# js43o/HifiDiff

Measured on AMD Instinct MI355X. Metric: faces/sec (whole node), 16→128 1000-step reverse diffusion, batch 64, higher is better.
Workload: dtype bf16

## Files before the change

hifidiff_amd/_lib.py:

```python
import ctypes
import os
import subprocess

import torch

_HERE = os.path.dirname(os.path.abspath(__file__))
LIB_PATH = os.path.join(_HERE, "libhifidiff_hip.so")
UNITS = [os.path.join(_HERE, "csrc", f) for f in ("hd_lib.hip", "hd_aux.hip", "hd_stages.hip", "hd_stages_rows.hip", "hd_strip.hip", "hd_dispatch_ln.hip", "hd_dispatch_lnface.hip", "hd_dispatch_bf16.hip", "hd_dispatch_misc.hip")]
SOURCES = UNITS + [os.path.join(_HERE, "csrc", f) for f in ("hd_gemm.hpp", "hd_dispatch.hpp", "hd_kernels.hpp", "hd_chain.hpp", "hd_conv.hpp", "hd_cr.hpp", "hd_vae.hpp", "hd_internal.hpp", "hd_faceset.hpp", "hd_stage_api.hpp", "hd_xcd.hpp", "hd_xcd2.hpp", "hd_face.hpp", "hd_strip.hpp", "hd_wide.hpp", "hd_end.hpp", "hd_color.hpp")]
HEADER = os.path.join(os.path.dirname(_HERE), "include", "hifidiff_hip.h")


def unit_deps(unit):
    import re
    seen, todo = [], [unit]
    while todo:
        f = os.path.normpath(todo.pop())
        if f in seen or not os.path.exists(f):
            continue
        seen.append(f)
        with open(f) as fh:
            for inc in re.findall(r'^\s*#include\s+"([^"]+)"', fh.read(), flags=re.M):
                todo.append(os.path.join(os.path.dirname(f), inc))
    return seen

EXPORTS = [
    "hd_create", "hd_create_unconditional", "hd_prepare_unconditional", "hd_cr_create", "hd_cr_forward", "hd_vae_create", "hd_vae_encode", "hd_vae_decode", "hd_destroy", "hd_last_error", "hd_load_weights", "hd_finalize_weights", "hd_prepare",
    "hd_prepare_from_priors", "hd_fpg", "hd_idc", "hd_eps", "hd_sample", "hd_sample_multistep", "hd_sample_rows", "hd_sample_rows_multistep", "hd_prepare_slots",
    "hd_pool_config", "hd_pool_prepare", "hd_pool_commit",
    "hd_sample_faces", "hd_sample_faces_multistep", "hd_sample_spans", "hd_mask_faces", "hd_guide_config", "hd_guide_faces", "hd_color_fix", "hd_preview_config", "hd_preview_read", "hd_scheduler_step",
    "hd_scheduler_step_multistep", "hd_num_ops", "hd_num_chains",
    "hd_debug_limit_ops", "hd_debug_op_name", "hd_debug_op_info", "hd_debug_read_op", "hd_debug_read", "hd_debug_write", "hd_set_option", "hd_get_option", "hd_check",
    "hd_set_profiling", "hd_get_profile",
]


class TensorDesc(ctypes.Structure):
    _fields_ = [("name", ctypes.c_char_p), ("data", ctypes.c_void_p), ("ndim", ctypes.c_int32),
                ("shape", ctypes.c_int64 * 4), ("is_device", ctypes.c_int32)]


class Schedule(ctypes.Structure):
    _fields_ = [("n_steps", ctypes.c_int32), ("timesteps", ctypes.POINTER(ctypes.c_float)),
                ("coef", ctypes.POINTER(ctypes.c_float))]


class ScheduleMS(ctypes.Structure):
    _fields_ = [("n_steps", ctypes.c_int32), ("timesteps", ctypes.POINTER(ctypes.c_float)),
                ("coef", ctypes.POINTER(ctypes.c_float))]


def build(force=False, verbose=False):
    if not force and os.path.exists(LIB_PATH):
        newest = max(os.path.getmtime(p) for p in SOURCES + [HEADER])
        if os.path.getmtime(LIB_PATH) >= newest:
            return LIB_PATH
    hipcc = os.environ.get("HIPCC", "/opt/rocm/bin/hipcc")
    flags = ["--offload-arch=gfx950", "-O3", "-std=c++17", "-fPIC", "-Wno-unused-result", "-Wno-unused-function"]
    objdir = os.path.join(_HERE, "csrc", "build")
    os.makedirs(objdir, exist_ok=True)
    objs = [os.path.join(objdir, os.path.splitext(os.path.basename(u))[0] + ".o") for u in UNITS]
    stale = [(u, o) for u, o in zip(UNITS, objs)
             if force or not os.path.exists(o) or os.path.getmtime(o) < max(os.path.getmtime(d) for d in unit_deps(u))]
    cmds = [[hipcc] + flags + ["-c", u, "-o", o] for u, o in stale]
    if verbose:
        for c in cmds:
            print(" ".join(c))
    procs = [subprocess.Popen(c) for c in cmds]
    failed = [u for (u, _), pr in zip(stale, procs) if pr.wait() != 0]
    if failed:
        raise subprocess.CalledProcessError(1, "hipcc -c " + " ".join(os.path.basename(f) for f in failed))
    link = [hipcc, "--offload-arch=gfx950", "-shared", "-fPIC", "-o", LIB_PATH] + objs
    if verbose:
        print(" ".join(link))
    subprocess.run(link, check=True)
    return LIB_PATH


_lib = None


def lib():
    global _lib
    if _lib is not None:
        return _lib
    if not os.path.exists(LIB_PATH):
        raise RuntimeError(f"{LIB_PATH} is not built (no CPU fallback exists); run __graft_entry__.build()")
    L = ctypes.CDLL(LIB_PATH)
    vp, i32, i64, u64 = ctypes.c_void_p, ctypes.c_int, ctypes.c_int64, ctypes.c_uint64
    L.hd_create.argtypes = [ctypes.POINTER(vp), i32, i32]
    L.hd_create_unconditional.argtypes = [ctypes.POINTER(vp), i32, i32]
    L.hd_prepare_unconditional.argtypes = [vp, i32, vp]
# ... 68 lines not shown
```

hifidiff_amd/csrc/hd_chain.hpp:

```cpp
#pragma once
#include "hd_gemm.hpp"

namespace hd {

struct ChainP {
    int M, hw, face0;
    const unsigned short* G;
    const float* pooled;
    const float* pool_part; int pool_nparts; float pool_scale; float* pooled_out;
    const float* X;
    const uint4 *Wsca, *W3, *W4, *W5;
    const float *bsca, *b3, *b4, *b5, *beta, *gamma;
    const float* film;
    int film_face_stride, film_gain_off, film_bias_off;
    float ln_eps;
    float* Xout;
    unsigned short* Xout16;
    float2* stats_out;
    unsigned short* outg16;
    const float *gate_c, *gate_s, *add_src;
#ifdef HD_STAMPS
    unsigned long long* stamps;
#endif
};
#ifdef HD_STAMPS
#define HD_CSTAMP(i) do { if (p.stamps && threadIdx.x == 0) p.stamps[(size_t)blockIdx.x * 8 + (i)] = __builtin_amdgcn_s_memrealtime(); } while (0)
#else
#define HD_CSTAMP(i) do { } while (0)
#endif

template <int C, int MT_ = 1>
struct ChainCfg {
    static constexpr int NT = C / 32;
    static constexpr int MT = MT_;
    static constexpr int WAVES = NT, THREADS = 64 * WAVES, BM = 32 * MT;
    static constexpr int TPW = 1;
    static constexpr int KS = C / 16;
    static constexpr int AROW = C * 2 + 16;
    static constexpr int YROW = C + 4;
    static constexpr int A1_OFF = 0;
    static constexpr int A2_OFF = A1_OFF + BM * AROW;
    static constexpr int Y_OFF = A2_OFF + BM * AROW;
    static constexpr int S_OFF = Y_OFF + BM * YROW * 4;
    static constexpr int GB_OFF = S_OFF + C * 4;
    static constexpr int SMEM = GB_OFF + 2 * C * 4;
    static_assert(TPW >= 1, "C must be a multiple of 128");
};

template <int C>
__device__ __forceinline__ void chain_load_b(const uint4* W, int tile, int lane, uint4* b) {
    const uint4* Wl = W + (size_t)tile * ChainCfg<C>::KS * 64 + lane;
#pragma unroll
    for (int ks = 0; ks < ChainCfg<C>::KS; ++ks) b[ks] = Wl[ks * 64];
}
template <int C, int MT>
__device__ __forceinline__ void chain_mma(const char* sA, const uint4* b, int lane, f32x16_t (&acc)[MT]) {
    const char* ap = sA + (lane & 31) * ChainCfg<C>::AROW + (lane >> 5) * 16;
#pragma unroll
    for (int mt = 0; mt < MT; ++mt)
#pragma unroll
        for (int i = 0; i < 16; ++i) acc[mt][i] = 0.f;
#pragma unroll
    for (int ks = 0; ks < ChainCfg<C>::KS; ++ks)
#pragma unroll
        for (int mt = 0; mt < MT; ++mt)
            acc[mt] = __builtin_amdgcn_mfma_f32_32x32x16_bf16(*reinterpret_cast<const bf16x8_t*>(ap + mt * 32 * ChainCfg<C>::AROW + ks * 32),
                                                              __builtin_bit_cast(bf16x8_t, b[ks]), acc[mt], 0, 0, 0);
}

#ifndef HD_CHAIN_OCC
#define HD_CHAIN_OCC 3
#endif
template <int C, int MT>
__global__ __launch_bounds__((ChainCfg<C, MT>::THREADS), (C == 128 && MT == 1 ? HD_CHAIN_OCC : 1)) void naf_chain_kernel(const ChainP p) {
    typedef ChainCfg<C, MT> K;
    extern __shared__ __attribute__((aligned(16))) char smem[];
    const int tid = threadIdx.x, lane = tid & 63, wave = tid >> 6;
    const int row0 = blockIdx.x * K::BM;
    const int face = row0 / p.hw;
    float* s_vec = reinterpret_cast<float*>(smem + K::S_OFF);
    float* gb = reinterpret_cast<float*>(smem + K::GB_OFF);
    float* yt = reinterpret_cast<float*>(smem + K::Y_OFF);
    const int tile = wave;
    const int col = tile * 32 + (lane & 31);
    const bool full = row0 + K::BM <= p.M;

    HD_CSTAMP(0);
    uint4 bw[K::KS], bw2[K::KS];
    chain_load_b<C>(p.Wsca, tile, lane, bw);
    chain_load_b<C>(p.W3, tile, lane, bw2);
    {
        const float* f = p.film + (size_t)(p.face0 + face) * p.film_face_stride;
        for (int k = tid; k < C; k += K::THREADS) { gb[k] = f[p.film_gain_off + k]; gb[C + k] = f[p.film_bias_off + k]; }
    }
    const float c_bsca = p.bsca[col], c_b3 = p.b3[col], c_beta = p.beta[col], c_b4a = p.b4[col], c_b4b = p.b4[col + C], c_b5 = p.b5[col],
                c_gamma = p.gamma[col];
    constexpr int kGIt = K::BM * (C / 8) / K::THREADS;
    static_assert(kGIt * K::THREADS == K::BM * (C / 8), "G tile / threads");
    uint4 gx[kGIt];
#pragma unroll
    for (int it = 0; it < kGIt; ++it) {
        const int u = tid + it * K::THREADS;
        const int rl = u / (C / 8), kq = u - rl * (C / 8);
        const int row = (full || row0 + rl < p.M) ? row0 + rl : row0;
        gx[it] = *reinterpret_cast<const uint4*>(p.G + (size_t)row * C + kq * 8);
    }
    {
        float* pl = yt;
        const float* pv = p.pooled + (size_t)face * C;
        if (p.pool_part) {
            const float* pp = p.pool_part + (size_t)face * p.pool_nparts * C;
            for (int k = tid; k < C; k += K::THREADS) {
                float v[8], s = 0.f;
#pragma unroll
                for (int b = 0; b < 8; ++b) v[b] = b < p.pool_nparts ? pp[b * C + k] : 0.f;
#pragma unroll
                for (int b = 0; b < 8; ++b) s += v[b];
                pl[k] = s * p.pool_scale;
                if (row0 == face * p.hw) p.pooled_out[(size_t)face * C + k] = pl[k];
            }
        } else {
            for (int k = tid; k < C; k += K::THREADS) pl[k] = pv[k];
        }
        __syncthreads();
        uint4 a[K::KS];
#pragma unroll
        for (int ks = 0; ks < K::KS; ++ks) {
            const float* q = pl + ks * 16 + 8 * (lane >> 5);
            const float4 v0 = *reinterpret_cast<const float4*>(q), v1 = *reinterpret_cast<const float4*>(q + 4);
            const uint4 row0 = make_uint4(pack2(v0.x, v0.y), pack2(v0.z, v0.w), pack2(v1.x, v1.y), pack2(v1.z, v1.w));
            a[ks] = (lane & 31) == 0 ? row0 : make_uint4(0, 0, 0, 0);
// ... 180 lines not shown
```

hifidiff_amd/csrc/hd_face.hpp:

```cpp
#pragma once
#ifndef HD_FACE_ROWS
#define HD_FACE_ROWS 0
#endif
#if HD_FACE_ROWS
#define HD_FACE_KERNEL naf_face_rows_stage_kernel
#define HD_FACE_LAUNCH launch_face_rows_stage
#else
#define HD_FACE_KERNEL naf_face_stage_kernel
#define HD_FACE_LAUNCH launch_face_stage
#endif
#include "hd_chain.hpp"
#include "hd_xcd.hpp"

namespace hd {

#ifdef HD_STAMPS
#define HD_FSTAMP(i) do { if (p.stamps && tid == 0) p.stamps[((size_t)blk * gridDim.x + blockIdx.x) * 8 + (i)] = __builtin_amdgcn_s_memrealtime(); } while (0)
#else
#define HD_FSTAMP(i) do { } while (0)
#endif

template <int C, int OWN_ = 32>
struct FaceCfg {
    static constexpr int S = (C == 128) ? 16 : 8;
    static constexpr int OWN = OWN_;
    static constexpr int HW = S * S, CL = HW / OWN, RI = OWN / S;
    static constexpr int NT = C / 32, THREADS = 64 * NT, KS = C / 16;
    static constexpr int ROWS = OWN + 2 * S, MT1 = (ROWS + 31) / 32;
    static constexpr int AROW = C * 2 + 16;
    static constexpr int XROW = C + 4;
    static constexpr int XT_OFF = 0;
    static constexpr int ALN_OFF = XT_OFF + OWN * XROW * 4;
    static constexpr int A1_OFF = ALN_OFF + 32 * AROW;
    static constexpr int T1_OFF = ALN_OFF + 64 * AROW;
    static constexpr int SV_OFF = T1_OFF + NT * MT1 * 32 * 32 * 4;
    static constexpr int GB_OFF = SV_OFF + C * 4;
    static constexpr int PL_OFF = GB_OFF + 4 * C * 4;
    static constexpr int PP_OFF = PL_OFF + C * 4;
    static constexpr int SMEM = PP_OFF + C * 4;
    static_assert(ROWS <= 64 && (OWN == 32 || OWN == 16) && RI >= 2 && RI % 2 == 0, "own + halo rows fit two MFMA row tiles; two lane halves share the image rows");
};

typedef __attribute__((address_space(1))) unsigned fs_gu32;

template <int C>
__device__ __forceinline__ void face_load_b(const uint4* W, int tile, int lane, uint4* b) {
#ifdef HD_STAMPS
    if (!W) return;
#endif
    const uint4* Wl = W + (size_t)tile * (C / 16) * 64 + lane;
#pragma unroll
    for (int ks = 0; ks < C / 16; ++ks) b[ks] = xs_ldg_u4(Wl + ks * 64);
}

template <int C, int OWN = 32>
__global__ __launch_bounds__((FaceCfg<C, OWN>::THREADS), 2) void HD_FACE_KERNEL(const FStageP p) {
    typedef FaceCfg<C, OWN> K;
    extern __shared__ __attribute__((aligned(16))) char smem[];
    __shared__ XBlockW s_blk[XS_MAXBLK];
    __shared__ unsigned s_abort, s_base;
    const int tid = threadIdx.x, lane = tid & 63, wave = __builtin_amdgcn_readfirstlane(tid >> 6);
    const int bid = blockIdx.x, xcd = bid & 7, jj = bid >> 3;
    const int fl = jj / K::CL, kk = jj - fl * K::CL;
    const int face = xcd * 8 + fl;
    if (face >= p.B) return;
    const int M = p.B * K::HW;
    const int row0 = face * K::HW + kk * OWN;
    const bool has_up = kk > 0, has_dn = kk < K::CL - 1;
    const int tile = wave, col = tile * 32 + (lane & 31);
    float* xt = reinterpret_cast<float*>(smem + K::XT_OFF);
    float* s_vec = reinterpret_cast<float*>(smem + K::SV_OFF);
    float* gb = reinterpret_cast<float*>(smem + K::GB_OFF);
    float* pooled = reinterpret_cast<float*>(smem + K::PL_OFF);
    float* poolp = reinterpret_cast<float*>(smem + K::PP_OFF);
    float* t1w = reinterpret_cast<float*>(smem + K::T1_OFF) + wave * K::MT1 * 32 * 32;

    {
        const unsigned* src = reinterpret_cast<const unsigned*>(p.blocks);
        unsigned* dst = reinterpret_cast<unsigned*>(s_blk);
        for (int i = tid; i < p.nblocks * (int)(sizeof(XBlockW) / 4); i += K::THREADS) dst[i] = src[i];
        if (tid == 0) {
            s_abort = __hip_atomic_load((fs_gu32*)p.abort_dev, __ATOMIC_RELAXED, __HIP_MEMORY_SCOPE_AGENT);
            s_base = __hip_atomic_load((fs_gu32*)(p.gstate + face * 16), __ATOMIC_RELAXED, __HIP_MEMORY_SCOPE_AGENT) * 64u;
        }
    }
    const __amdgpu_buffer_rsrc_t rs_X = __builtin_amdgcn_make_buffer_rsrc(p.X, 0, (int)((size_t)M * C * 4), 0x00020000);
    const __amdgpu_buffer_rsrc_t rs_PP = __builtin_amdgcn_make_buffer_rsrc(p.pool_part, 0, p.B * K::CL * C * 4, 0x00020000);
    fs_gu32* flags = (fs_gu32*)(p.flags + face * 16);

    bool intro = false;
    float* hb = reinterpret_cast<float*>(smem + K::T1_OFF);
    if constexpr (C == 128 && OWN == 32) intro = p.intro_lat != nullptr;
    bool from_x = !intro;
    if constexpr (C == 256 && OWN == 16) from_x = p.down_A == nullptr;
    if (from_x) {
// ... 124 lines not shown
                uint4 v = make_uint4(0, 0, 0, 0);
                if (ok) {
                    const int l0row = face * 256 + (2 * y1 + (tap >> 1)) * 16 + 2 * x1 + (tap & 1);
                    v = *reinterpret_cast<const uint4*>(p.down_A + (size_t)l0row * 128 + q * 8);
                }
                *reinterpret_cast<uint4*>(sA + r * DROW + (tap * 128 + q * 8) * 2) = v;
            }
            uint4 wa[16], wb[16];
            {
                const uint4* Wl = p.down_W + (size_t)tile * 32 * 64 + lane;
#pragma unroll
                for (int ks = 0; ks < 16; ++ks) wa[ks] = xs_ldg_u4(Wl + ks * 64);
#pragma unroll
                for (int ks = 0; ks < 16; ++ks) wb[ks] = xs_ldg_u4(Wl + (16 + ks) * 64);
            }
            const float bias = p.down_b[col];
            __syncthreads();
            f32x16_t acc;
#pragma unroll
            for (int i = 0; i < 16; ++i) acc[i] = 0.f;
            const char* ap = sA + (lane & 31) * DROW + (lane >> 5) * 16;
#pragma unroll
            for (int ks = 0; ks < 16; ++ks)
                acc = __builtin_amdgcn_mfma_f32_32x32x16_bf16(*reinterpret_cast<const bf16x8_t*>(ap + ks * 32), __builtin_bit_cast(bf16x8_t, wa[ks]), acc, 0, 0, 0);
#pragma unroll
            for (int ks = 0; ks < 16; ++ks)
                acc = __builtin_amdgcn_mfma_f32_32x32x16_bf16(*reinterpret_cast<const bf16x8_t*>(ap + (16 + ks) * 32), __builtin_bit_cast(bf16x8_t, wb[ks]), acc, 0, 0, 0);
#pragma unroll
            for (int i = 0; i < 16; ++i) {
                const int r = (i & 3) + 8 * (i >> 2) + 4 * (lane >> 5);
                float* dst = r < OWN ? xt + r * K::XROW : hb + (r - OWN) * K::XROW;
                dst[col] = acc[i] + bias;
            }
        }
    }
    __syncthreads();
    const unsigned base = s_base;
    bool dead = false;

    auto publish = [&](unsigned value) __attribute__((always_inline)) {
        asm volatile("s_waitcnt vmcnt(0)" ::: "memory");
        __syncthreads();
        if (tid == 0) __hip_atomic_store(flags + kk, value, __ATOMIC_RELAXED, __HIP_MEMORY_SCOPE_AGENT);
    };
    auto poll = [&](unsigned value, unsigned code) __attribute__((always_inline)) {
        if (wave == 0) {
            for (unsigned spins = 0;; ++spins) {
                const unsigned v = lane < K::CL ? __hip_atomic_load(flags + lane, __ATOMIC_RELAXED, __HIP_MEMORY_SCOPE_AGENT) : value;
                if (__all((int)(v - value) >= 0)) break;
                if (spins > XS_SPINS) {
                    if (lane == 0) {
                        s_abort = 1u;
                        __hip_atomic_store((fs_gu32*)p.abort_dev, code, __ATOMIC_RELAXED, __HIP_MEMORY_SCOPE_AGENT);
                        __hip_atomic_store((fs_gu32*)p.tmo, code, __ATOMIC_RELAXED, __HIP_MEMORY_SCOPE_SYSTEM);
                    }
                    break;
                }
                __builtin_amdgcn_s_sleep(1);
            }
        }
    };
    auto wait_for = [&](unsigned value, unsigned code) __attribute__((always_inline)) {
        if (wave == 0) {
            for (unsigned spins = 0;; ++spins) {
                const unsigned v = lane < K::CL ? __hip_atomic_load(flags + lane, __ATOMIC_RELAXED, __HIP_MEMORY_SCOPE_AGENT) : value;
                const bool inject = p.test_abort >= 1000 && (int)(code & 0xffu) == p.test_abort - 1000 && face == 0;
                if (!inject && __all((int)(v - value) >= 0)) break;
                if (spins > XS_SPINS || inject) {
                    if (lane == 0) {
                        s_abort = 1u;
                        __hip_atomic_store((fs_gu32*)p.abort_dev, code, __ATOMIC_RELAXED, __HIP_MEMORY_SCOPE_AGENT);
                        __hip_atomic_store((fs_gu32*)p.tmo, code, __ATOMIC_RELAXED, __HIP_MEMORY_SCOPE_SYSTEM);
                    }
                    break;
                }
                __builtin_amdgcn_s_sleep(1);
            }
        }
        __syncthreads();
        dead = s_abort != 0u;
    };
    constexpr int V4 = C / 64;
    auto ln_row = [&](const float4 (&v)[V4], const float* g, const float* b, char* dst_row, bool valid) __attribute__((always_inline)) {
        const int l16 = lane & 15;
        float sum = 0.f;
#pragma unroll
        for (int i = 0; i < V4; ++i) sum += (v[i].x + v[i].y) + (v[i].z + v[i].w);
        const float mean = row16_sum(sum) * (1.0f / C);
        float q = 0.f;
#pragma unroll
        for (int i = 0; i < V4; ++i) {
            const float d0 = v[i].x - mean, d1 = v[i].y - mean, d2 = v[i].z - mean, d3 = v[i].w - mean;
            q += (d0 * d0 + d1 * d1) + (d2 * d2 + d3 * d3);
        }
        const float rstd = 1.0f / sqrtf(row16_sum(q) * (1.0f / C) + p.ln_eps);
        const float nmr = -mean * rstd;
#pragma unroll
        for (int i = 0; i < V4; ++i) {
            const int k = 4 * l16 + 64 * i;
            const float x4[4] = {v[i].x, v[i].y, v[i].z, v[i].w};
            float o[4];
#pragma unroll
            for (int e = 0; e < 4; ++e) {
                const float xq = bf16_bits_to_f32(f32_to_bf16_bits(x4[e]));
                o[e] = valid ? fmaf(fmaf(xq, rstd, nmr), g[k + e], b[k + e]) : 0.f;
            }
            *reinterpret_cast<uint2*>(dst_row + k * 2) = make_uint2(pack2(o[0], o[1]), pack2(o[2], o[3]));
        }
    };

    const int nb_run = p.block_limit < 0 ? 0 : (p.block_limit > 0 && p.block_limit < p.nblocks) ? p.block_limit : p.nblocks;
    uint4 bw[K::KS], bw2[K::KS];
    for (int blk = 0; blk < nb_run; ++blk) {
        const XBlockW& B = s_blk[blk];
        HD_FSTAMP(0);
        float4 gbv = make_float4(0.f, 0.f, 0.f, 0.f);
        const int gi = tid - 64;
        static_assert(K::THREADS - 64 >= C, "one float4 of the FiLM rows per thread of waves 1..");
#if HD_FACE_ROWS
        if (gi >= 0 && gi < C) gbv = *reinterpret_cast<const float4*>(p.film + (size_t)face * p.film_face_stride + B.film_off + 4 * gi);
#else
        if (gi >= 0 && gi < C) gbv = *reinterpret_cast<const float4*>(p.film + B.film_off + 4 * gi);
#endif
        face_load_b<C>(B.w1, tile, lane, bw);
        if constexpr (C == 128) face_load_b<C>(B.w1, tile + K::NT, lane, bw2);
        constexpr bool kEarly = C == 128;
        float c_b1a = 0.f, c_b1b = 0.f, dwa[9], dwb[9], dba = 0.f, dbb = 0.f;
        auto load_dw_consts = [&]() __attribute__((always_inline)) {
            c_b1a = xs_ldg_f(B.b1 + col); c_b1b = xs_ldg_f(B.b1 + col + C);
#pragma unroll
            for (int t = 0; t < 9; ++t) { dwa[t] = xs_ldg_f(B.dw_w + (size_t)t * 2 * C + col); dwb[t] = xs_ldg_f(B.dw_w + (size_t)t * 2 * C + col + C); }
            dba = xs_ldg_f(B.dw_b + col); dbb = xs_ldg_f(B.dw_b + col + C);
        };
        if constexpr (kEarly) load_dw_consts();
        if (blk > 0) poll(base + 2u * (unsigned)(blk - 1) + 2u, 0x200u + (unsigned)blk);
        if (gi >= 0 && gi < C) *reinterpret_cast<float4*>(gb + 4 * gi) = gbv;
        __syncthreads();
        if (s_abort) return;
        {
            const int l16 = lane & 15;
            constexpr int ROWS = K::ROWS;
            constexpr int HRI = (ROWS - OWN + K::NT * 4 - 1) / (K::NT * 4);
            constexpr int HSH = (K::NT * 4 - OWN % (K::NT * 4)) % (K::NT * 4);
            float4 hv[HRI][V4];
            bool hok[HRI];
#pragma unroll
            for (int hi = 0; hi < HRI; ++hi) {
                const int r = OWN + hi * K::NT * 4 + (wave * 4 + (lane >> 4) + HSH) % (K::NT * 4);
                const bool up = r < OWN + K::S;
                hok[hi] = r < ROWS && (up ? has_up : has_dn);
                const int grow = up ? row0 - K::S + (r - OWN) : row0 + OWN + (r - OWN - K::S);
                const int gr = hok[hi] ? grow : row0;
                if (intro && blk == 0) {
                    const int hr = r < ROWS ? r - OWN : 0;
#pragma unroll
                    for (int i = 0; i < V4; ++i) hv[hi][i] = *reinterpret_cast<const float4*>(hb + hr * K::XROW + 4 * l16 + 64 * i);
                } else {
#pragma unroll
                    for (int i = 0; i < V4; ++i) {
                        const xs_u32x4 raw = __builtin_amdgcn_raw_buffer_load_b128(rs_X, (gr * C + 4 * l16 + 64 * i) * 4, 0, 16);
                        hv[hi][i] = make_float4(__uint_as_float(raw.x), __uint_as_float(raw.y), __uint_as_float(raw.z), __uint_as_float(raw.w));
                    }
                }
            }
            for (int r = wave * 4 + (lane >> 4); r < OWN; r += K::NT * 4) {
                float4 v[V4];
#pragma unroll
                for (int i = 0; i < V4; ++i) v[i] = *reinterpret_cast<const float4*>(xt + r * K::XROW + 4 * l16 + 64 * i);
                ln_row(v, gb + C, gb, smem + K::ALN_OFF + r * K::AROW, true);
            }
#pragma unroll
            for (int hi = 0; hi < HRI; ++hi) {
                const int r = OWN + hi * K::NT * 4 + (wave * 4 + (lane >> 4) + HSH) % (K::NT * 4);
                if (r < ROWS) ln_row(hv[hi], gb + C, gb, smem + K::ALN_OFF + r * K::AROW, hok[hi]);
            }
        }
        __syncthreads();
        HD_FSTAMP(1);
        f32x16_t acc_a[K::MT1], acc_b[K::MT1];
        chain_mma<C, K::MT1>(smem + K::ALN_OFF, bw, lane, acc_a);
        if constexpr (kEarly) {
            chain_mma<C, K::MT1>(smem + K::ALN_OFF, bw2, lane, acc_b);
            face_load_b<C>(B.wsca, tile, lane, bw);
            face_load_b<C>(B.w3, tile, lane, bw2);
        } else {
            face_load_b<C>(B.w1, tile + K::NT, lane, bw);
            load_dw_consts();
        }
        HD_FSTAMP(2);
        constexpr int NU = (K::RI / 2) * K::S;
        float u1[NU], u2[NU];
        auto dw_half = [&](const f32x16_t (&acc)[K::MT1], float bias1, const float (&w)[9], float bias2, float (&u)[NU]) __attribute__((always_inline)) {
            __builtin_amdgcn_wave_barrier();
#pragma unroll
            for (int mt = 0; mt < K::MT1; ++mt)
#pragma unroll
                for (int i = 0; i < 16; ++i) {
                    const int r = mt * 32 + (i & 3) + 8 * (i >> 2) + 4 * (lane >> 5);
                    t1w[r * 32 + (lane & 31)] = acc[mt][i] + bias1;
                }
            __builtin_amdgcn_wave_barrier();
            const int j = lane & 31, h = lane >> 5;
            constexpr int S = K::S, IRL = K::RI / 2;
#pragma unroll
            for (int q = 0; q < IRL; ++q) {
                const int ir = h * IRL + q;
                float v[3][S + 2];
#pragma unroll
                for (int rr = 0; rr < 3; ++rr) { v[rr][0] = 0.f; v[rr][S + 1] = 0.f; }
                const bool up_in = ir > 0, dn_in = ir < K::RI - 1;
                const bool up_ok = up_in || has_up, dn_ok = dn_in || has_dn;
                const int up_base = up_in ? (ir - 1) * S : OWN, dn_base = dn_in ? (ir + 1) * S : OWN + S;
#pragma unroll
                for (int x = 0; x < S; ++x) {
                    v[0][x + 1] = up_ok ? t1w[(up_base + x) * 32 + j] : 0.f;
                    v[1][x + 1] = t1w[(ir * S + x) * 32 + j];
                    v[2][x + 1] = dn_ok ? t1w[(dn_base + x) * 32 + j] : 0.f;
                }
#pragma unroll
                for (int x = 0; x < S; ++x) {
                    float a = bias2;
#pragma unroll
                    for (int rr = 0; rr < 3; ++rr) {
                        a = fmaf(w[rr * 3], v[rr][x], a); a = fmaf(w[rr * 3 + 1], v[rr][x + 1], a); a = fmaf(w[rr * 3 + 2], v[rr][x + 2], a);
                    }
                    u[q * S + x] = a;
                }
            }
        };
        dw_half(acc_a, c_b1a, dwa, dba, u1);
        if constexpr (!kEarly) {
            chain_mma<C, K::MT1>(smem + K::ALN_OFF, bw, lane, acc_b);
            face_load_b<C>(B.wsca, tile, lane, bw);
        }
        dw_half(acc_b, c_b1b, dwb, dbb, u2);
        if constexpr (!kEarly) face_load_b<C>(B.w3, tile, lane, bw2);
        __syncthreads();
        {
            const int j = lane & 31, h = lane >> 5;
            constexpr int IRL = K::RI / 2;
            float rsum = 0.f;
#pragma unroll
            for (int q = 0; q < IRL; ++q)
#pragma unroll
                for (int x = 0; x < K::S; ++x) {
                    const float g = u1[q * K::S + x] * u2[q * K::S + x];
                    rsum += g;
                    const int r = (h * IRL + q) * K::S + x;
                    *reinterpret_cast<unsigned short*>(smem + K::A1_OFF + r * K::AROW + (tile * 32 + j) * 2) = f32_to_bf16_bits(g);
                }
            const float other = __shfl_xor(rsum, 32);
            if (h == 0) poolp[tile * 32 + j] = rsum + other;
        }
        __syncthreads();
        HD_FSTAMP(3);
        if (tid < C / 4) {
            const float4 v = *reinterpret_cast<const float4*>(poolp + 4 * tid);
            const xs_u32x4 x = {__float_as_uint(v.x), __float_as_uint(v.y), __float_as_uint(v.z), __float_as_uint(v.w)};
            __builtin_amdgcn_raw_buffer_store_b128(x, rs_PP, ((face * K::CL + kk) * C + 4 * tid) * 4, 0, 16);
        }
        publish(base + 2u * (unsigned)blk + 1u);
        wait_for(base + 2u * (unsigned)blk + 1u, 0x300u + (unsigned)blk);
        if (dead) return;
        if (tid < C / 4) {
            float4 s = make_float4(0.f, 0.f, 0.f, 0.f);
#pragma unroll
            for (int m = 0; m < K::CL; ++m) {
                const xs_u32x4 raw = __builtin_amdgcn_raw_buffer_load_b128(rs_PP, ((face * K::CL + m) * C + 4 * tid) * 4, 0, 16);
                s.x += __uint_as_float(raw.x); s.y += __uint_as_float(raw.y); s.z += __uint_as_float(raw.z); s.w += __uint_as_float(raw.w);
            }
            const float inv = 1.0f / (float)K::HW;
            *reinterpret_cast<float4*>(pooled + 4 * tid) = make_float4(s.x * inv, s.y * inv, s.z * inv, s.w * inv);
        }
        const float c_bsca = xs_ldg_f(B.bsca + col), c_b3 = xs_ldg_f(B.b3 + col), c_beta = xs_ldg_f(B.beta + col), c_b4a = xs_ldg_f(B.b4 + col),
                    c_b4b = xs_ldg_f(B.b4 + col + C), c_b5 = xs_ldg_f(B.b5 + col), c_gamma = xs_ldg_f(B.gamma + col);
        __syncthreads();
        HD_FSTAMP(4);
        {
            f32x16_t acc;
#pragma unroll
            for (int i = 0; i < 16; ++i) acc[i] = 0.f;
#pragma unroll
            for (int ks = 0; ks < K::KS; ++ks) {
                const float* q = pooled + ks * 16 + 8 * (lane >> 5);
                const float4 v0 = *reinterpret_cast<const float4*>(q), v1 = *reinterpret_cast<const float4*>(q + 4);
                const uint4 r0 = make_uint4(pack2(v0.x, v0.y), pack2(v0.z, v0.w), pack2(v1.x, v1.y), pack2(v1.z, v1.w));
                const uint4 a = (lane & 31) == 0 ? r0 : make_uint4(0, 0, 0, 0);
                acc = __builtin_amdgcn_mfma_f32_32x32x16_bf16(__builtin_bit_cast(bf16x8_t, a), __builtin_bit_cast(bf16x8_t, bw[ks]), acc, 0, 0, 0);
            }
            if (lane < 32) s_vec[col] = acc[0] + c_bsca;
        }
        face_load_b<C>(B.w4, tile, lane, bw);
        __syncthreads();
        for (int u = tid; u < OWN * (C / 8); u += K::THREADS) {
            const int r = u / (C / 8), q = u - r * (C / 8);
            uint4* gp = reinterpret_cast<uint4*>(smem + K::A1_OFF + r * K::AROW + q * 16);
            float v[8];
            unpack8(*gp, v);
#pragma unroll
            for (int i = 0; i < 8; ++i) v[i] *= s_vec[q * 8 + i];
            *gp = pack8(v);
        }
        __syncthreads();
        {
            f32x16_t acc[1];
            chain_mma<C, 1>(smem + K::A1_OFF, bw2, lane, acc);
            face_load_b<C>(B.w4, tile + K::NT, lane, bw2);
#pragma unroll
            for (int i = 0; i < OWN / 2; ++i) {
                const int r = (i & 3) + 8 * (i >> 2) + 4 * (lane >> 5);
                xt[r * K::XROW + col] = xt[r * K::XROW + col] + (acc[0][i] + c_b3) * c_beta;
            }
        }
        __syncthreads();
        {
            const int l16 = lane & 15;
            for (int r = wave * 4 + (lane >> 4); r < OWN; r += K::NT * 4) {
                float4 v[V4];
#pragma unroll
                for (int i = 0; i < V4; ++i) v[i] = *reinterpret_cast<const float4*>(xt + r * K::XROW + 4 * l16 + 64 * i);
                ln_row(v, gb + 3 * C, gb + 2 * C, smem + K::ALN_OFF + r * K::AROW, true);
            }
        }
        __syncthreads();
        {
            f32x16_t a1[1], a2[1];
            chain_mma<C, 1>(smem + K::ALN_OFF, bw, lane, a1);
            chain_mma<C, 1>(smem + K::ALN_OFF, bw2, lane, a2);
            face_load_b<C>(B.w5, tile, lane, bw);
#pragma unroll
            for (int i = 0; i < OWN / 2; ++i) {
                const int r = (i & 3) + 8 * (i >> 2) + 4 * (lane >> 5);
                *reinterpret_cast<unsigned short*>(smem + K::A1_OFF + r * K::AROW + col * 2) = f32_to_bf16_bits((a1[0][i] + c_b4a) * (a2[0][i] + c_b4b));
            }
        }
// ... 70 lines not shown
```

hifidiff_amd/csrc/hd_strip.hpp:

```cpp
#pragma once
#include <type_traits>
#include "hd_chain.hpp"
#include "hd_stage_api.hpp"

namespace hd {

template <int C_, int S_>
struct StripCfg {
    static constexpr int C = C_, S = S_, HW = S * S;
    static constexpr int RI = 4, OWN = RI * S, ROWS = OWN + 2 * S, MT = ROWS / 32;
    static constexpr int NSTRIP = S / RI;
    static constexpr int NT = C / 32, KS = C / 16;
    static constexpr int WAVES = 4, THREADS = 64 * WAVES, CG = NT / WAVES;
    static constexpr int RT = 32 / S, NB = S / 8, RPI = S / 2;
    static constexpr int AROW = ChainCfg<C>::AROW;
    static constexpr int ALN_OFF = 0;
    static constexpr int SMEM = ALN_OFF + ROWS * AROW;
    static constexpr int V = C / 128;
    static_assert((S == 32 || S == 16) && ROWS % 32 == 0 && (C == 128 || C == 256) && NSTRIP <= 8, "shapes this kernel is written for");
    static_assert((OWN * (32 * WAVES / 8)) % THREADS == 0 && ROWS % (THREADS / 16) == 0 && NT % WAVES == 0, "copy-out and LayerNorm passes");
};

__device__ __forceinline__ float strip_other_half(float v) { return __shfl_xor(v, 32); }

template <class K>
__device__ __forceinline__ void strip_mma(const char* sA, const uint4* b, int lane, f32x16_t (&acc)[K::MT]) {
    const char* ap = sA + (lane & 31) * K::AROW + (lane >> 5) * 16;
#pragma unroll
    for (int mt = 0; mt < K::MT; ++mt)
#pragma unroll
        for (int i = 0; i < 16; ++i) acc[mt][i] = 0.f;
    typedef unsigned u32x4_t __attribute__((ext_vector_type(4)));
    u32x4_t a[2][K::MT];
#pragma unroll
    for (int mt = 0; mt < K::MT; ++mt) a[0][mt] = *reinterpret_cast<const u32x4_t*>(ap + mt * 32 * K::AROW);
#pragma unroll
    for (int ks = 0; ks < K::KS; ++ks) {
        if (ks + 1 < K::KS) {
#pragma unroll
            for (int mt = 0; mt < K::MT; ++mt) a[(ks + 1) & 1][mt] = *reinterpret_cast<const u32x4_t*>(ap + mt * 32 * K::AROW + (ks + 1) * 32);
        }
#pragma unroll
        for (int mt = 0; mt < K::MT; ++mt) {
            asm volatile("" : "+v"(a[ks & 1][mt]) :: "memory");
            acc[mt] = __builtin_amdgcn_mfma_f32_32x32x16_bf16(__builtin_bit_cast(bf16x8_t, a[ks & 1][mt]), __builtin_bit_cast(bf16x8_t, b[ks]), acc[mt], 0, 0, 0);
        }
    }
}

template <int C, int S>
__global__ __launch_bounds__((StripCfg<C, S>::THREADS), 2) void naf_strip_dwgate_kernel(const StripP p) {
    typedef StripCfg<C, S> K;
    extern __shared__ __attribute__((aligned(16))) char smem[];
    const int tid = threadIdx.x, lane = tid & 63, wave = __builtin_amdgcn_readfirstlane(tid >> 6);
    const int lid = (gridDim.x & 7) == 0 ? (blockIdx.x & 7) * (gridDim.x >> 3) + (blockIdx.x >> 3) : blockIdx.x;
    const int cg = lid % K::CG, sid = lid / K::CG;
    const int face = sid / K::NSTRIP, kk = sid - face * K::NSTRIP;
    const bool has_up = kk > 0, has_dn = kk < K::NSTRIP - 1;
    const int row_first = face * K::HW + kk * K::OWN - K::S;
    const int tile = cg * K::WAVES + wave, col = tile * 32 + (lane & 31);

    uint4 bw[K::KS];
    chain_load_b<C>(p.W1, tile, lane, bw);
    {
        const int l16 = lane & 15, g16 = tid >> 4;
        constexpr int RG = K::THREADS / 16, PASSES = K::ROWS / RG;
        const float* f = p.film + (size_t)(p.face0 + face) * p.film_face_stride;
        float gn[K::V][8], bs[K::V][8];
#pragma unroll
        for (int v = 0; v < K::V; ++v) {
            const int k = 8 * l16 + 128 * v;
            const float4 g0 = *reinterpret_cast<const float4*>(f + p.film_gain_off + k), g1 = *reinterpret_cast<const float4*>(f + p.film_gain_off + k + 4);
            const float4 b0 = *reinterpret_cast<const float4*>(f + p.film_bias_off + k), b1 = *reinterpret_cast<const float4*>(f + p.film_bias_off + k + 4);
            gn[v][0] = g0.x; gn[v][1] = g0.y; gn[v][2] = g0.z; gn[v][3] = g0.w; gn[v][4] = g1.x; gn[v][5] = g1.y; gn[v][6] = g1.z; gn[v][7] = g1.w;
            bs[v][0] = b0.x; bs[v][1] = b0.y; bs[v][2] = b0.z; bs[v][3] = b0.w; bs[v][4] = b1.x; bs[v][5] = b1.y; bs[v][6] = b1.z; bs[v][7] = b1.w;
        }
        uint4 raw[PASSES][K::V];
        float2 part[PASSES];
        const int np = p.stats_np;
#pragma unroll
        for (int it = 0; it < PASSES; ++it) {
            const int r = it * RG + g16;
            const bool ok = (r >= K::S || has_up) && (r < K::S + K::OWN || has_dn);
            const int row = ok ? row_first + r : row_first + K::S;
#pragma unroll
            for (int v = 0; v < K::V; ++v) raw[it][v] = *reinterpret_cast<const uint4*>(p.Xb + (size_t)row * C + 8 * l16 + 128 * v);
            part[it] = l16 < np ? p.stats_in[(size_t)row * np + l16] : make_float2(0.f, 0.f);
        }
        const float inv_np = 1.0f / (float)np, cnt = (float)p.stats_cnt;
#pragma unroll
        for (int it = 0; it < PASSES; ++it) {
            const int r = it * RG + g16;
            const bool ok = (r >= K::S || has_up) && (r < K::S + K::OWN || has_dn);
            const float mean = row16_sum(part[it].x) * inv_np;
            const float d = part[it].x - mean;
            const float q = l16 < np ? fmaf(cnt * d, d, part[it].y) : 0.f;
            const float var = row16_sum(q) * (inv_np / cnt);
            float rstd = __frsqrt_rn(var + p.ln_eps), mu = -mean * rstd;
            asm volatile("" : "+v"(rstd), "+v"(mu));
#pragma unroll
            for (int v = 0; v < K::V; ++v) {
                float x[8];
                unpack8(raw[it][v], x);
#pragma unroll
                for (int e = 0; e < 8; ++e) x[e] = fmaf(fmaf(x[e], rstd, mu), gn[v][e], bs[v][e]);
                *reinterpret_cast<uint4*>(smem + K::ALN_OFF + r * K::AROW + 16 * l16 + 256 * v) = ok ? pack8(x) : make_uint4(0, 0, 0, 0);
            }
// ... 110 lines not shown
```

Baseline: 66.99.

## Compute face depthwise conv directly from MFMA accumulators via lane shuffles

Adds a register-resident depthwise 3x3 path for the face kernel. It reads the MFMA accumulator layout in place and exchanges edge pixels between the lane halves with xor-32 shuffles, so the LDS round trip and the wave barrier are no longer needed. A compile-time map (FaceDwMap) gives each lane's tile, register and partner slots, and the gate write and pooling are remapped to the new pixel ordering. The LDS path stays for C==256 with OWN==32 or when the macro is set, and an asm barrier on the lane index is added for C==256. This trades LDS traffic for extra shuffles and register pressure.

```diff
diff --git a/hifidiff_amd/_lib.py b/hifidiff_amd/_lib.py
--- a/hifidiff_amd/_lib.py
+++ b/hifidiff_amd/_lib.py
@@ -7,7 +7,7 @@
 _HERE = os.path.dirname(os.path.abspath(__file__))
 LIB_PATH = os.path.join(_HERE, "libhifidiff_hip.so")
 UNITS = [os.path.join(_HERE, "csrc", f) for f in ("hd_lib.hip", "hd_aux.hip", "hd_stages.hip", "hd_stages_rows.hip", "hd_strip.hip", "hd_dispatch_ln.hip", "hd_dispatch_lnface.hip", "hd_dispatch_bf16.hip", "hd_dispatch_misc.hip")]
-SOURCES = UNITS + [os.path.join(_HERE, "csrc", f) for f in ("hd_gemm.hpp", "hd_dispatch.hpp", "hd_kernels.hpp", "hd_chain.hpp", "hd_conv.hpp", "hd_cr.hpp", "hd_vae.hpp", "hd_internal.hpp", "hd_faceset.hpp", "hd_stage_api.hpp", "hd_xcd.hpp", "hd_xcd2.hpp", "hd_face.hpp", "hd_strip.hpp", "hd_wide.hpp", "hd_end.hpp", "hd_color.hpp")]
+SOURCES = UNITS + [os.path.join(_HERE, "csrc", f) for f in ("hd_gemm.hpp", "hd_dispatch.hpp", "hd_kernels.hpp", "hd_chain.hpp", "hd_conv.hpp", "hd_cr.hpp", "hd_vae.hpp", "hd_internal.hpp", "hd_faceset.hpp", "hd_stage_api.hpp", "hd_xcd.hpp", "hd_xcd2.hpp", "hd_face.hpp", "hd_face_dw.hpp", "hd_strip.hpp", "hd_wide.hpp", "hd_end.hpp", "hd_color.hpp")]
 HEADER = os.path.join(os.path.dirname(_HERE), "include", "hifidiff_hip.h")
 
 
diff --git a/hifidiff_amd/csrc/hd_chain.hpp b/hifidiff_amd/csrc/hd_chain.hpp
--- a/hifidiff_amd/csrc/hd_chain.hpp
+++ b/hifidiff_amd/csrc/hd_chain.hpp
@@ -47,6 +47,8 @@
     static_assert(TPW >= 1, "C must be a multiple of 128");
 };
 
+__device__ __forceinline__ float strip_other_half(float v) { return __shfl_xor(v, 32); }
+
 template <int C>
 __device__ __forceinline__ void chain_load_b(const uint4* W, int tile, int lane, uint4* b) {
     const uint4* Wl = W + (size_t)tile * ChainCfg<C>::KS * 64 + lane;
diff --git a/hifidiff_amd/csrc/hd_face.hpp b/hifidiff_amd/csrc/hd_face.hpp
--- a/hifidiff_amd/csrc/hd_face.hpp
+++ b/hifidiff_amd/csrc/hd_face.hpp
@@ -11,6 +11,11 @@
 #endif
 #include "hd_chain.hpp"
 #include "hd_xcd.hpp"
+#include "hd_face_dw.hpp"
+
+#ifndef HD_FACE_DW_LDS
+#define HD_FACE_DW_LDS 0
+#endif
 
 namespace hd {
 
@@ -301,7 +306,8 @@
     };
     constexpr int V4 = C / 64;
     auto ln_row = [&](const float4 (&v)[V4], const float* g, const float* b, char* dst_row, bool valid) __attribute__((always_inline)) {
-        const int l16 = lane & 15;
+        int l16 = lane & 15;
+        if constexpr (C == 256) asm volatile("" : "+v"(l16));
         float sum = 0.f;
 #pragma unroll
         for (int i = 0; i < V4; ++i) sum += (v[i].x + v[i].y) + (v[i].z + v[i].w);
@@ -407,9 +413,54 @@
             load_dw_consts();
         }
         HD_FSTAMP(2);
-        constexpr int NU = (K::RI / 2) * K::S;
+        typedef hdi::FaceDwMap<K::S, OWN> DW;
+        constexpr bool kDwLds = HD_FACE_DW_LDS || (C == 256 && OWN == 32);
+        constexpr int NU = DW::RI * DW::RPI;
+        static_assert(NU == (K::RI / 2) * K::S, "both forms hold the same number of pixels per lane");
         float u1[NU], u2[NU];
-        auto dw_half = [&](const f32x16_t (&acc)[K::MT1], float bias1, const float (&w)[9], float bias2, float (&u)[NU]) __attribute__((always_inline)) {
+        const bool hi = lane >= 32;
+        auto dw_half_acc = [&](f32x16_t (&acc)[K::MT1], float bias1, const float (&w)[9], float bias2, float (&u)[NU]) __attribute__((always_inline)) {
+#pragma unroll
+            for (int y = -1; y <= DW::RI; ++y) {
+                const bool ok = DW::row_ok(y, has_up, has_dn);
+#pragma unroll
+                for (int k = 0; k < DW::RPI; ++k) {
+                    const int m = DW::tile(y), i = DW::reg(y, k);
+                    acc[m][i] = ok ? acc[m][i] + bias1 : 0.f;
+                }
+            }
+            float ex[DW::RI + 2][DW::NX];
+            auto edges = [&](int y) __attribute__((always_inline)) {
+#pragma unroll
+                for (int s = 0; s < DW::NX; ++s) {
+                    const float lo = acc[DW::tile(y)][DW::reg(y, DW::slot_send(s, 0))], up = acc[DW::tile(y)][DW::reg(y, DW::slot_send(s, 1))];
+                    ex[y + 1][s] = strip_other_half(hi ? up : lo);
+                }
+            };
+            auto tap = [&](int y, int k, int dx) __attribute__((always_inline)) -> float {
+                const typename DW::Src s0 = DW::tap(k, 0, dx), s1 = DW::tap(k, 1, dx);
+                if (s0.kind == DW::OWN_REG) return acc[DW::tile(y)][DW::reg(y, s0.k)];
+                const float v0 = s0.kind == DW::ZERO ? 0.f : ex[y + 1][s0.slot < 0 ? 0 : s0.slot];
+                const float v1 = s1.kind == DW::ZERO ? 0.f : ex[y + 1][s1.slot < 0 ? 0 : s1.slot];
+                return hi ? v1 : v0;
+            };
+            edges(-1); edges(0);
+#pragma unroll
+            for (int y = 0; y < DW::RI; ++y) {
+                edges(y + 1);
+#pragma unroll
+                for (int k = 0; k < DW::RPI; ++k) {
+                    float a = bias2;
+#pragma unroll
+                    for (int rr = 0; rr < 3; ++rr) {
+                        const int yy = y + rr - 1;
+                        a = fmaf(w[rr * 3], tap(yy, k, -1), a); a = fmaf(w[rr * 3 + 1], acc[DW::tile(yy)][DW::reg(yy, k)], a); a = fmaf(w[rr * 3 + 2], tap(yy, k, 1), a);
+                    }
+                    u[y * DW::RPI + k] = a;
+                }
+            }
+        };
+        auto dw_half_lds = [&](const f32x16_t (&acc)[K::MT1], float bias1, const float (&w)[9], float bias2, float (&u)[NU]) __attribute__((always_inline)) {
             __builtin_amdgcn_wave_barrier();
 #pragma unroll
             for (int mt = 0; mt < K::MT1; ++mt)
@@ -446,6 +497,9 @@
                     u[q * S + x] = a;
                 }
             }
+        };
+        auto dw_half = [&](f32x16_t (&acc)[K::MT1], float bias1, const float (&w)[9], float bias2, float (&u)[NU]) __attribute__((always_inline)) {
+            if constexpr (kDwLds) dw_half_lds(acc, bias1, w, bias2, u); else dw_half_acc(acc, bias1, w, bias2, u);
         };
         dw_half(acc_a, c_b1a, dwa, dba, u1);
         if constexpr (!kEarly) {
@@ -455,7 +509,7 @@
         dw_half(acc_b, c_b1b, dwb, dbb, u2);
         if constexpr (!kEarly) face_load_b<C>(B.w3, tile, lane, bw2);
         __syncthreads();
-        {
+        if constexpr (kDwLds) {
             const int j = lane & 31, h = lane >> 5;
             constexpr int IRL = K::RI / 2;
             float rsum = 0.f;
@@ -468,8 +522,21 @@
                     const int r = (h * IRL + q) * K::S + x;
                     *reinterpret_cast<unsigned short*>(smem + K::A1_OFF + r * K::AROW + (tile * 32 + j) * 2) = f32_to_bf16_bits(g);
                 }
-            const float other = __shfl_xor(rsum, 32);
+            const float other = strip_other_half(rsum);
             if (h == 0) poolp[tile * 32 + j] = rsum + other;
+        } else {
+            const int h = lane >> 5;
+            float rsum = 0.f;
+#pragma unroll
+            for (int y = 0; y < DW::RI; ++y)
+#pragma unroll
+                for (int k = 0; k < DW::RPI; ++k) {
+                    const float g = u1[y * DW::RPI + k] * u2[y * DW::RPI + k];
+                    rsum += g;
+                    *reinterpret_cast<unsigned short*>(smem + K::A1_OFF + DW::gate_row(y, k, h) * K::AROW + col * 2) = f32_to_bf16_bits(g);
+                }
+            const float other = strip_other_half(rsum);
+            if (!hi) poolp[col] = rsum + other;
         }
         __syncthreads();
         HD_FSTAMP(3);
diff --git a/hifidiff_amd/csrc/hd_face_dw.hpp b/hifidiff_amd/csrc/hd_face_dw.hpp
--- /dev/null
+++ b/hifidiff_amd/csrc/hd_face_dw.hpp
@@ -0,0 +1,37 @@
+#pragma once
+
+namespace hdi {
+
+template <int S_, int OWN_>
+struct FaceDwMap {
+    static constexpr int S = S_, OWN = OWN_, RI = OWN / S;
+    static constexpr int NB = S / 8, RPI = S / 2;
+    static constexpr int NX = 2 * NB - 1;
+    static_assert((S == 8 || S == 16) && OWN % S == 0 && RI >= 1 && OWN + 2 * S <= 64, "own + halo rows in at most two 32-row tiles");
+
+    static constexpr int tile_row(int i, int h) { return (i & 3) + 8 * (i >> 2) + 4 * h; }
+    static constexpr int row_base(int y) { return y < 0 ? OWN : y < RI ? y * S : OWN + S; }
+    static constexpr int tile(int y) { return row_base(y) / 32; }
+    static constexpr int reg(int y, int k) { return (row_base(y) % 32) / 2 + k; }
+    static constexpr int px(int k, int h) { return 8 * (k >> 2) + 4 * h + (k & 3); }
+    static constexpr int k_of(int x) { return 4 * (x >> 3) + (x & 3); }
+    static constexpr int h_of(int x) { return (x >> 2) & 1; }
+    static constexpr int gate_row(int y, int k, int h) { return y * S + px(k, h); }
+    static constexpr bool row_ok(int y, bool has_up, bool has_dn) { return y < 0 ? has_up : y < RI ? true : has_dn; }
+
+    static constexpr int slot_recv(int s, int h) { return s < NB ? (h == 0 ? 4 * s : 4 * s + 3) : (h == 0 ? 4 * (s - NB) + 3 : 4 * (s - NB + 1)); }
+    static constexpr int slot_send(int s, int h) { return slot_recv(s, 1 - h); }
+
+    enum Kind { ZERO, OWN_REG, PARTNER };
+    struct Src { Kind kind; int k; int slot; };
+    static constexpr Src tap(int k, int h, int dx) {
+        const int x = px(k, h) + dx;
+        if (x < 0 || x >= S) return Src{ZERO, 0, -1};
+        if (h_of(x) == h) return Src{OWN_REG, k_of(x), -1};
+        const int b = k >> 2;
+        const int s = dx < 0 ? (h == 0 ? NB + b - 1 : b) : (h == 0 ? b : NB + b);
+        return Src{PARTNER, k_of(x), s};
+    }
+};
+
+}
diff --git a/hifidiff_amd/csrc/hd_strip.hpp b/hifidiff_amd/csrc/hd_strip.hpp
--- a/hifidiff_amd/csrc/hd_strip.hpp
+++ b/hifidiff_amd/csrc/hd_strip.hpp
@@ -21,8 +21,6 @@
     static_assert((OWN * (32 * WAVES / 8)) % THREADS == 0 && ROWS % (THREADS / 16) == 0 && NT % WAVES == 0, "copy-out and LayerNorm passes");
 };
 
-__device__ __forceinline__ float strip_other_half(float v) { return __shfl_xor(v, 32); }
-
 template <class K>
 __device__ __forceinline__ void strip_mma(const char* sA, const uint4* b, int lane, f32x16_t (&acc)[K::MT]) {
     const char* ap = sA + (lane & 31) * K::AROW + (lane >> 5) * 16;
```

New measurement: 67.13, median of 2. No clear change (+0.2%).
